# ViktorLiang/GW-Depth

Hardware: AMD Instinct MI355X
Metric: images/sec (train fwd+bwd) 480x640 bs=8/GPU (higher is better)
Workload: dtype bf16; 1 GPU; GW-Depth full model (res50 + DETR 6+6 + 4-scale ReferTransformer + decoder) fwd+17 losses+bwd+clip+AdamW, 480x640, bs=8/GPU, dropout 0.1; global_batch=8, parallelism=dp1, launch=hipgraph, graph_segments=1, grad_buckets=8

## Files before the change

### gw_depth_amd/hip.py

```python
import ctypes
import os

import torch

_HERE = os.path.dirname(os.path.abspath(__file__))
LIB_PATH = os.environ.get("GWD_LIB") or os.path.join(_HERE, "libgwdepth_hip.so")

F32, BF16 = 0, 1
ACT_NONE, ACT_RELU, ACT_GELU, ACT_ELU, ACT_SIGMOID = 0, 1, 2, 3, 4
WS_INORM_GELU, WS_RESAMPLE_BWD, WS_EVAL, WS_PLANE = 0, 1, 2, 3
GATHER_CONV, GATHER_TRANSPOSED, GATHER_UPSAMPLED = 0, 1, 2
RESAMPLE_BILINEAR_AC, RESAMPLE_NEAREST = 0, 1

ENTRY_POINTS = [
    "gwd_version", "gwd_arch", "gwd_conv_forward", "gwd_conv_wgrad", "gwd_weight_prep", "gwd_act_backward",
    "gwd_colsum", "gwd_layernorm_forward", "gwd_layernorm_backward", "gwd_softmax_forward",
    "gwd_softmax_backward", "gwd_silog_sums", "gwd_silog_backward", "gwd_seg_ce_sum", "gwd_seg_ce_backward",
    "gwd_sqnorm", "gwd_adamw_step", "gwd_resample_forward", "gwd_resample_backward", "gwd_avgpool_forward",
    "gwd_avgpool_backward", "gwd_winattn_forward", "gwd_winattn_backward", "gwd_tokattn_forward",
    "gwd_tokattn_backward", "gwd_tokattn_pair_forward", "gwd_tokattn_pair_backward", "gwd_upsample_taps_collapse", "gwd_upsample_taps_fold", "gwd_certain_sample", "gwd_lsap", "gwd_window_map", "gwd_window_map_multi",
    "gwd_inorm_gelu_forward", "gwd_inorm_gelu_backward", "gwd_weight_prep_batch",
    "gwd_point_sample_forward", "gwd_point_sample_backward", "gwd_act_backward_colsum", "gwd_resample_backward_sep",
    "gwd_softmax_masked_forward", "gwd_softmax_scaled_backward", "gwd_query_workspace", "gwd_eval_accumulate", "gwd_colsum_batch", "gwd_conv_wgrad_batch",
    "gwd_conv_wgrad_takes_bias",
    "gwd_plane_loss_forward", "gwd_plane_loss_backward", "gwd_collate",
    "gwd_anchor_depth_forward", "gwd_anchor_depth_backward", "gwd_mha_flash_forward", "gwd_mha_flash_backward",
    "gwd_ref_scores_forward", "gwd_ref_scores_backward", "gwd_ref_mix_forward", "gwd_ref_mix_backward", "gwd_unpad_add_batch", "gwd_stem_pack", "gwd_stem_forward", "gwd_pos_sine", "gwd_silog_finalize", "gwd_psp_pool_forward", "gwd_psp_pool_backward",
    "gwd_match_cost", "gwd_set_losses_forward", "gwd_set_losses_backward", "gwd_set_losses_focal_forward", "gwd_set_losses_focal_backward", "gwd_resample_u8_pass", "gwd_gather2d", "gwd_point_sample_backward_gather", "gwd_point_sample_framed_forward", "gwd_point_sample_framed_backward", "gwd_stride_place", "gwd_color_adjust", "gwd_bmm",
    "gwd_dense_postprocess", "gwd_line_postprocess", "gwd_line_score",
    "gwd_dense_postprocess_resized",
    "gwd_resample_u8_pass_batch", "gwd_gather2d_batch", "gwd_color_adjust_batch",
]


class HipUnavailable(RuntimeError):
    pass


class ConvDesc(ctypes.Structure):
    _fields_ = [("x", ctypes.c_void_p), ("w", ctypes.c_void_p), ("y", ctypes.c_void_p), ("z", ctypes.c_void_p),
                ("scale", ctypes.c_void_p), ("shift", ctypes.c_void_p), ("residual", ctypes.c_void_p),
                ("zero_page", ctypes.c_void_p), ("mult", ctypes.c_void_p), ("gate", ctypes.c_void_p)] + \
               [(n, ctypes.c_int32) for n in ("B", "Hi", "Wi", "Cin", "Ho", "Wo", "Cout", "KH", "KW", "stride", "pad",
                                              "gather", "Hv", "Wv", "act")] + \
               [("act_scale", ctypes.c_float), ("dtype", ctypes.c_int32), ("gate_act", ctypes.c_int32),
                ("ln_mean", ctypes.c_void_p), ("ln_rstd", ctypes.c_void_p), ("ln_C", ctypes.c_int32), ("reserved", ctypes.c_int32),
                ("dbias", ctypes.c_void_p)]


class BmmDesc(ctypes.Structure):
    _fields_ = [("a", ctypes.c_void_p), ("b", ctypes.c_void_p), ("c", ctypes.c_void_p)] + \
               [(n, ctypes.c_int64) for n in ("a_sb0", "a_sb1", "a_ld", "b_sb0", "b_sb1", "b_ld", "c_sb0", "c_sb1", "c_ld")] + \
               [(n, ctypes.c_int32) for n in ("M", "N", "K", "nb0", "nb1", "a_kmajor", "b_kmajor", "c_is_f32_accumulate", "splits")] + \
               [("alpha", ctypes.c_float), ("dtype", ctypes.c_int32)]


class PrepJob(ctypes.Structure):
    _fields_ = [("w", ctypes.c_void_p), ("row_scale", ctypes.c_void_p), ("w_fwd", ctypes.c_void_p), ("w_dgrad", ctypes.c_void_p),
                ("N", ctypes.c_int32), ("taps", ctypes.c_int32), ("C", ctypes.c_int32), ("block0", ctypes.c_int32),
                ("Np", ctypes.c_int32), ("Cg", ctypes.c_int32), ("Cgp", ctypes.c_int32), ("reserved", ctypes.c_int32)]


class UnpadJob(ctypes.Structure):
    _fields_ = [("src", ctypes.c_void_p), ("dst", ctypes.c_void_p), ("N", ctypes.c_int32), ("taps", ctypes.c_int32), ("G", ctypes.c_int32),
# ... 158 lines not shown
        L.gwd_ref_mix_backward.argtypes = [vp, vp, vp, vp, vp, i32, i32, i32, i32, i32, i32, vp]
        L.gwd_tokattn_forward.argtypes = [sp] * 4 + [i64, i32, i32, f32, i32, vp]
        L.gwd_tokattn_backward.argtypes = [sp] * 7 + [i64, i32, i32, f32, i32, vp]
        L.gwd_upsample_taps_collapse.argtypes = [vp, vp, i32, i32, i32, vp]
        L.gwd_upsample_taps_fold.argtypes = [vp, vp, i32, i32, vp]
        L.gwd_tokattn_pair_forward.argtypes = [sp] * 6 + [i64, i32, i32, f32, i32, vp]
        L.gwd_tokattn_pair_backward.argtypes = [sp] * 10 + [i64, i32, i32, f32, i32, vp]
        L.gwd_certain_sample.argtypes = [vp, vp, vp, i32, i32, i32, i32, i32, vp, i32, i32, vp]
        L.gwd_lsap.argtypes = [vp, vp, vp, i32, i32, i32, i32, i32, vp]
        L.gwd_inorm_gelu_forward.argtypes = [vp, vp, vp, vp, vp, i64, i64, i32, i32, ctypes.c_float, i32, vp]
        L.gwd_inorm_gelu_backward.argtypes = [vp, vp, vp, vp, vp, i64, i64, i32, i32, i32, vp]
        L.gwd_query_workspace.argtypes = [i32, ctypes.POINTER(ctypes.c_int64), i32]
        L.gwd_query_workspace.restype = ctypes.c_int64
        L.gwd_eval_accumulate.argtypes = [vp, vp, vp, i64, i64, i64, vp, vp, vp, vp, vp, i32, i64, f32, f32, i32, i32, vp]
        L.gwd_dense_postprocess.argtypes = [vp, vp, i64, i64, i64, vp, vp, vp, vp, i32, i32, i32, f32, f32, i32, i32, vp]
        L.gwd_dense_postprocess_resized.argtypes = [vp, vp, i64, i64, i64, vp, vp, i32, vp, vp, vp] + [i32] * 5 + [f32, f32, i32, i32, vp]
        L.gwd_line_postprocess.argtypes = [vp] * 7 + [i32, i32, i32, f32, vp]
        dp = ctypes.POINTER(ctypes.c_double)
        L.gwd_line_score.argtypes = [vp] * 5 + [dp, i32, dp, i32] + [vp] * 4 + [i32] * 4 + [i64, i64, vp]
        L.gwd_softmax_masked_forward.argtypes = [vp, vp, vp, i64, i32, i64, ctypes.c_float, i32, vp]
        L.gwd_softmax_scaled_backward.argtypes = [vp, vp, vp, i64, i32, ctypes.c_float, i32, vp]
        L.gwd_resample_backward_sep.argtypes = [vp, vp, vp] + [i32] * 9 + [vp]
        L.gwd_act_backward_colsum.argtypes = [vp, vp, vp, vp, i64, i32, i32, ctypes.c_float, vp, i32, vp]
        L.gwd_point_sample_forward.argtypes = [vp, vp, vp, i32, i32, i32, i32, i32, i32, i32, vp]
        L.gwd_point_sample_backward.argtypes = [vp, vp, vp, i32, i32, i32, i32, i32, i32, i32, vp]
        L.gwd_point_sample_backward_gather.argtypes = [vp, vp, vp, i32, i32, i32, i32, i32, i32, i32, vp]
        L.gwd_point_sample_framed_forward.argtypes = [vp, vp, vp, i32, i32, i32, i32, i32, i32, i32, i32, i32, vp]
        L.gwd_point_sample_framed_backward.argtypes = [vp, vp, vp, i32, i32, i32, i32, i32, i32, i32, i32, i32, vp]
        L.gwd_weight_prep_batch.argtypes = [vp, i32, i32, vp, vp]
        L.gwd_window_map.argtypes = [vp, vp, vp, i32, i32, i32, i32, i32, i32, i32, vp]
        L.gwd_window_map_multi.argtypes = [vp, vp, vp, vp, i32, i32, i32, i32, i32, i32, i32, vp]
        L.gwd_sqnorm.argtypes = [vp, vp, i64, vp]
        L.gwd_adamw_step.argtypes = [vp, vp, vp, vp, vp, vp, i64] + [f32] * 9 + [vp]

    @staticmethod
    def _stream(*tensors):
        for t in tensors:
            if t is not None and not t.is_cuda:
                raise HipUnavailable("gw_depth_amd ops run on a HIP device only (got a %s tensor); "
                                     "there is no CPU path" % t.device)
        return ctypes.c_void_p(torch.cuda.current_stream().cuda_stream)

    @staticmethod
    def _check(rc, what):
        if rc != 0:
            raise RuntimeError("%s failed with status %d" % (what, rc))

    def workspace_bytes(self, op, *dims):
        arr = (ctypes.c_int64 * len(dims))(*[int(d) for d in dims])
        n = self.lib.gwd_query_workspace(op, arr, len(dims))
        if n < 0:
            raise ValueError("gwd_query_workspace(%d, %r) -> %d" % (op, dims, n))
        return n

    def version(self):
        return self.lib.gwd_version()

    @staticmethod
    def _desc(x, w, y, dims, z=None, scale=None, shift=None, residual=None, stride=1, pad=0,
              gather=GATHER_CONV, virt=(0, 0), act=ACT_NONE, act_scale=1.0, mult=None, gate=None, gate_act=ACT_NONE, ln=None,
              zero_page=True, dbias=None):
        B, Hi, Wi, Cin, Ho, Wo, Cout, KH, KW = dims
        d = ConvDesc()
        d.x, d.w, d.y, d.z = _ptr(x), _ptr(w), _ptr(y), _ptr(z)
        d.scale, d.shift, d.residual = _ptr(scale), _ptr(shift), _ptr(residual)
        d.zero_page = _zero_page(x.device) if zero_page else None
# ... 381 lines not shown
                                                 dtype_code(ra), self._stream(ra, ref_v, q_new, att)), "gwd_ref_mix_forward")

    def ref_mix_backward(self, att, ref_v, g, d_ra, d_ref_v, H):
        B, T, R = att.shape[0], att.shape[1], att.shape[2]
        self._check(self.lib.gwd_ref_mix_backward(_ptr(att), _ptr(ref_v), _ptr(g), _ptr(d_ra), _ptr(d_ref_v), B, T, R, H,
                                                  ref_v.shape[2] // H, dtype_code(att), self._stream(att, ref_v, g, d_ra, d_ref_v)),
                    "gwd_ref_mix_backward")

    def tokattn_forward(self, q, k, v, o, scale):
        W, N, H, _ = q.shape
        s = [_strided(t) for t in (q, k, v, o)]
        self._check(self.lib.gwd_tokattn_forward(*[ctypes.byref(x) for x in s], W, H, k.shape[3], scale, dtype_code(q),
                                                 self._stream(q, k, v, o)), "gwd_tokattn_forward")

    def tokattn_backward(self, q, k, v, go, gq, gk, gv, scale):
        W, N, H, _ = q.shape
        s = [_strided(t) for t in (q, k, v, go, gq, gk, gv)]
        self._check(self.lib.gwd_tokattn_backward(*[ctypes.byref(x) for x in s], W, H, k.shape[3], scale, dtype_code(q),
                                                  self._stream(q, go, gq)), "gwd_tokattn_backward")

    def upsample_taps_collapse(self, w, wk):
        Cout, KH, KW, Cin = w.shape
        if (KH, KW) != (3, 3) or tuple(wk.shape) != (Cin, 4, 4, Cout) or w.dtype != torch.float32 or not (w.is_contiguous() and wk.is_contiguous()):
            raise ValueError("upsample_taps_collapse: w (Cout,3,3,Cin) fp32 -> wk (Cin,4,4,Cout), both contiguous")
        self._check(self.lib.gwd_upsample_taps_collapse(_ptr(w), _ptr(wk), Cout, Cin, dtype_code(wk), self._stream(w, wk)), "gwd_upsample_taps_collapse")

    def upsample_taps_fold(self, D, dw):
        Cout, KH, KW, Cin = dw.shape
        if (KH, KW) != (3, 3) or tuple(D.shape) != (Cin, 4, 4, Cout) or D.dtype != torch.float32 or dw.dtype != torch.float32 \
                or not (D.is_contiguous() and dw.is_contiguous()):
            raise ValueError("upsample_taps_fold: D (Cin,4,4,Cout) fp32 -> dw (Cout,3,3,Cin) fp32, both contiguous")
        self._check(self.lib.gwd_upsample_taps_fold(_ptr(D), _ptr(dw), Cout, Cin, self._stream(D, dw)), "gwd_upsample_taps_fold")

    def tokattn_pair_forward(self, q, q2, k, v, o, o2, scale):
        W, N, H, _ = q.shape
        s = [_strided(t) for t in (q, q2, k, v, o, o2)]
        rc = self.lib.gwd_tokattn_pair_forward(*[ctypes.byref(x) for x in s], W, H, k.shape[3], scale, dtype_code(q),
                                               self._stream(q, q2, k, v, o, o2))
        if rc == -4:
            return False
        self._check(rc, "gwd_tokattn_pair_forward")
        return True

    def tokattn_pair_backward(self, q, q2, k, v, go, go2, gq, gq2, gk, gv, scale):
        W, N, H, _ = q.shape
        s = [_strided(t) for t in (q, q2, k, v, go, go2, gq, gq2, gk, gv)]
        rc = self.lib.gwd_tokattn_pair_backward(*[ctypes.byref(x) for x in s], W, H, k.shape[3], scale, dtype_code(q),
                                                self._stream(q, go, gq))
        if rc == -4:
            return False
        self._check(rc, "gwd_tokattn_pair_backward")
        return True

    def certain_sample(self, small, large, coords, edges, sample_num):
        B, _, hs, ws = small.shape
        H, W = large.shape[-2:]
        self._check(self.lib.gwd_certain_sample(_ptr(small), _ptr(large), _ptr(coords), B, hs, ws, H, W, _ptr(edges),
                                                edges.numel() - 1, sample_num, self._stream(small, large, coords)),
                    "gwd_certain_sample")

    def bmm(self, a, b, c, M, N, K, a_kmajor=False, b_kmajor=False, alpha=1.0, accumulate=False, splits=1):
        for t in (a, b, c):
            if t.dim() != 4 or t.stride(3) != 1:
                raise ValueError("bmm: 4-D operands with unit inner stride expected")
        nb0, nb1 = c.shape[0], c.shape[1]
        d = BmmDesc()
# ... 209 lines not shown
```

### gw_depth_amd/model.py

```python
import math
import os

import torch
import torch.nn.functional as F
from torch import nn

from . import ops
from .layers import Conv, FrozenBN, LayerNorm, Linear, Mlp, MlpNorm, Seq
from .ops import ACT_ELU, ACT_GELU, ACT_NONE, ACT_RELU, ACT_SIGMOID

WS = 7
HEADS = 16
DEFAULT_FP32_STAGES = ()


class NestedTensor:

    def __init__(self, tensors, mask):
        self.tensors, self.mask = tensors, mask

    def to(self, device):
        return NestedTensor(self.tensors.to(device), None if self.mask is None else self.mask.to(device))

    def decompose(self):
# ... 539 lines not shown

    def __init__(self, c, pools=(16, 8, 4, 2)):
        super().__init__()
        self.pools = pools
        self.firstconv = Seq(_0=ConvLn(c, c, 3), _2=ConvLn(c, 2 * c, 3))
        c2 = 2 * c
        self.layer1 = nn.Sequential(PyrBlock(c2))
        self.layer2 = nn.Sequential(PyrBlock(c2), PyrBlock(c2))
        self.layer3 = nn.Sequential(PyrBlock(c2), PyrBlock(c2))
        self.layer4 = nn.Sequential(PyrBlock(c2))
        for i in range(1, 5):
            setattr(self, f"branch{i}", Seq(_1=ConvLn(c2, c2, 3)))
        self.lastconv = Seq(_0=ConvLn(5 * c2, 2 * c2, 3), _2=Conv(2 * c2, c, 1))

    FORCE_PAD = False

    def padded_width(self, ref):
        c = self.firstconv[0].conv.weight.shape[0]
        if c % 8 and ((ref.dtype == torch.bfloat16 and ref.is_cuda) or self.FORCE_PAD):
            return (c + 31) // 32 * 32
        return c

    def forward(self, x):
        c = self.firstconv[0].conv.weight.shape[0]
        if x.shape[-1] != c:
            return self.forward_padded(x, c)
        x = self.firstconv[2](self.firstconv[0](x, True), True)
        x = self.layer3(self.layer2(self.layer1(x)))
        B, H, W, C = x.shape
        if H < self.pools[0] or W < self.pools[0]:
            x = F.pad(x, (0, 0, 0, max(self.pools[0] - W, 0), 0, max(self.pools[0] - H, 0)))
        x, pooled = ops.psp_pools(x, self.pools)
        ys = [getattr(self, f"branch{i}")[1](p, True) for i, p in enumerate(pooled, start=1)]
        x = self.lastconv[0](ops.pyramid_concat(x, ys), True)
        return ops.conv2d(x, self.lastconv[2].weight)

    def forward_padded(self, x, c):
        r32 = lambda n: (n + 31) // 32 * 32
        cp, c2, c2p, c4, c4p = r32(c), 2 * c, r32(2 * c), 4 * c, r32(4 * c)
        if x.shape[-1] != cp:
            raise ValueError("PyramidLayer: a map of %d or %d channels expected, got %d" % (c, cp, x.shape[-1]))
        x = self.firstconv[2](self.firstconv[0](x, True, geom=(cp, c, cp)), True, geom=(c2p, c, cp))
        g2 = (c2p, c2, c2p)
        for layer in (self.layer1, self.layer2, self.layer3):
            for blk in layer:
                x = blk(x, g2)
        B, H, W, C = x.shape
        if H < self.pools[0] or W < self.pools[0]:
            x = F.pad(x, (0, 0, 0, max(self.pools[0] - W, 0), 0, max(self.pools[0] - H, 0)))
        x, pooled = ops.psp_pools(x, self.pools)
        ys = [getattr(self, f"branch{i}")[1](p, True, geom=g2) for i, p in enumerate(pooled, start=1)]
        x = self.lastconv[0](ops.pyramid_concat(x, ys), True, geom=(c4p, c2, c2p))
        return ops.conv2d_padded(x, self.lastconv[2].weight, 0, (cp, c4, c4p))


class PointBasedPred(nn.Module):

    def __init__(self, dim, tdim, point_num):
        super().__init__()
        self.dim = dim
        self.pre_proj = Linear(dim + tdim, dim)
        self.refer_proj = Linear(dim, dim * 2)
        self.pyramid = PyramidLayer(point_num)

    def forward(self, x, dtok, pre_depth, coords, H, W, pos):
        B = x.shape[0]
        xg_xr = self.refer_proj(self.pre_proj(torch.cat([x, dtok], dim=-1)))
# ... 279 lines not shown
```

### gw_depth_amd/ops.py

```python
import bisect
import os

import torch
import torch.nn.functional as F

from . import hip
from .hip import (ACT_ELU, ACT_GELU, ACT_NONE, ACT_RELU, ACT_SIGMOID, GATHER_CONV, GATHER_TRANSPOSED,
                  GATHER_UPSAMPLED)

__all__ = ["conv2d", "linear", "layer_norm", "softmax_lastdim", "silog_loss", "seg_cross_entropy",
           "ACT_NONE", "ACT_RELU", "ACT_GELU", "ACT_ELU", "ACT_SIGMOID"]


def _lib():
    return hip.library()


class WeightCache:

    def __init__(self, persistent=(), frozen=False):
        self.frozen = bool(frozen)
        self._derived = {}
        self.ranges = sorted((int(a), int(b)) for a, b in persistent)
        self._starts, self._ends, self._merged_from = [], [], -1
# ... 1101 lines not shown
        shapes = []
        for k, y in enumerate(ys):
            y = y.contiguous()
            if y.shape[0] != B or y.shape[3] != C:
                raise ValueError("pyramid_concat: branch %d has shape %r" % (k, tuple(y.shape)))
            lib.resample_forward(y, out[..., (k + 1) * C:(k + 2) * C], B, y.shape[1], y.shape[2], H, W, C, hip.RESAMPLE_BILINEAR_AC)
            shapes.append((y.shape[1], y.shape[2]))
        ctx.cfg = (B, H, W, C, shapes)
        return out

    @staticmethod
    def backward(ctx, g):
        lib = _lib()
        B, H, W, C, shapes = ctx.cfg
        g = g.contiguous()
        grads = [g[..., :C]]
        for k, (h, w) in enumerate(shapes):
            gk = g[..., (k + 1) * C:(k + 2) * C]
            gy = torch.empty((B, h, w, C), dtype=g.dtype, device=g.device)
            tmp = torch.empty(lib.workspace_bytes(hip.WS_RESAMPLE_BWD, B, H, w, C) // 4, dtype=torch.float32, device=g.device)
            if not lib.resample_backward_sep(gk, tmp, gy, B, h, w, H, W, C, hip.RESAMPLE_BILINEAR_AC):
                lib.resample_backward(gk.contiguous(), gy, B, h, w, H, W, C, hip.RESAMPLE_BILINEAR_AC)
            grads.append(gy)
        return tuple(grads)


def pyramid_concat(x, ys):
    C = x.shape[-1]
    if C % 8 or not ys:
        return torch.cat([x] + [upsample_bilinear_ac(y, x.shape[1:3]) for y in ys], dim=-1)
    return _PyramidCatFn.apply(x, *ys)


def upsample_bilinear_ac(x, size):
    return _ResampleFn.apply(x, tuple(size), hip.RESAMPLE_BILINEAR_AC)


def upsample_nearest(x, size):
    return _ResampleFn.apply(x, tuple(size), hip.RESAMPLE_NEAREST)


class _AvgPoolFn(torch.autograd.Function):
    @staticmethod
    def forward(ctx, x, k):
        x = x.contiguous()
        B, H, W, C = x.shape
        y = torch.empty((B, H // k, W // k, C), dtype=x.dtype, device=x.device)
        _lib().avgpool_forward(x, y, B, H, W, C, k)
        ctx.cfg = (B, H, W, C, k)
        return y

    @staticmethod
    def backward(ctx, gy):
        B, H, W, C, k = ctx.cfg
        gx = torch.empty((B, H, W, C), dtype=gy.dtype, device=gy.device)
        _lib().avgpool_backward(gy.contiguous(), gx, B, H, W, C, k)
        return gx, None


def avg_pool(x, k):
    return _AvgPoolFn.apply(x, int(k))


class _WinAttnPackedFn(torch.autograd.Function):

    @staticmethod
# ... 601 lines not shown
```

### include/gwdepth.h

```cpp
#ifndef GWDEPTH_H
#define GWDEPTH_H
#include <stdint.h>

#ifdef __cplusplus
extern "C" {
#endif

#define GWD_VERSION 10

enum { GWD_F32 = 0, GWD_BF16 = 1 };
enum { GWD_ACT_NONE = 0, GWD_ACT_RELU = 1, GWD_ACT_GELU = 2, GWD_ACT_ELU = 3, GWD_ACT_SIGMOID = 4 };
enum {
    GWD_GATHER_CONV = 0,
    GWD_GATHER_TRANSPOSED = 1,
    GWD_GATHER_UPSAMPLED = 2
};

typedef struct {
    const void *x;
    const void *w;
    void *y;
    void *z;
    const float *scale;
    const float *shift;
// ... 183 lines not shown
    const float *src;
    float *dst;
    int32_t N, taps, G, Cg, Cgp;
    int32_t block0;
} gwd_unpad_job;
int gwd_unpad_add_batch(const gwd_unpad_job *jobs, int32_t n_jobs, void *stream);

int gwd_inorm_gelu_forward(const void *a, const void *u, void *y, float *part, float *stat, int64_t B, int64_t L, int32_t C,
                           int32_t S, float eps, int32_t dtype, void *stream);
int gwd_inorm_gelu_backward(const void *gy, const void *u, const float *stat, float *part, void *du, int64_t B, int64_t L,
                            int32_t C, int32_t S, int32_t dtype, void *stream);

int gwd_window_map(const void *src, void *dst, const void *residual, int32_t B, int32_t H, int32_t W, int32_t C, int32_t shift,
                   int32_t gather, int32_t dtype, void *stream);
#define GWD_WINMAP_JOBS 4
int gwd_window_map_multi(const void *const *src, void *const *dst, const void *const *residual, const int32_t *C, int32_t n,
                         int32_t B, int32_t H, int32_t W, int32_t shift, int32_t gather, int32_t dtype, void *stream);

enum { GWD_RESAMPLE_BILINEAR_AC = 0, GWD_RESAMPLE_NEAREST = 1 };
int gwd_resample_forward(const void *x, void *y, int32_t B, int32_t Hs, int32_t Ws, int32_t Ho, int32_t Wo,
                         int32_t C, int32_t mode, int32_t ldy, int32_t dtype, void *stream);
int gwd_resample_backward(const void *gy, void *gx, int32_t B, int32_t Hs, int32_t Ws, int32_t Ho, int32_t Wo,
                          int32_t C, int32_t mode, const void *gate, int32_t gate_act, int32_t dtype, void *stream);
int gwd_resample_backward_sep(const void *gy, float *tmp, void *gx, int32_t B, int32_t Hs, int32_t Ws, int32_t Ho, int32_t Wo,
                              int32_t C, int32_t mode, int32_t ldg, int32_t dtype, void *stream);

int gwd_stride_place(const void *src, const void *residual, void *dst, int32_t B, int32_t H, int32_t W, int32_t Ho, int32_t Wo, int32_t C,
                     int32_t stride, int32_t dtype, void *stream);

int gwd_psp_pool_forward(const void *x, void *p16, void *p8, void *p4, void *p2, int32_t B, int32_t H, int32_t W, int32_t C,
                         int32_t dtype, void *stream);
int gwd_psp_pool_backward(const void *g_pass, const void *g16, const void *g8, const void *g4, const void *g2, void *gx, int32_t B,
                          int32_t H, int32_t W, int32_t C, int32_t ldg, int32_t dtype, void *stream);
int gwd_avgpool_forward(const void *x, void *y, int32_t B, int32_t H, int32_t W, int32_t C, int32_t k,
                        int32_t dtype, void *stream);
int gwd_avgpool_backward(const void *gy, void *gx, int32_t B, int32_t H, int32_t W, int32_t C, int32_t k,
                         int32_t dtype, void *stream);

int gwd_sqnorm(const float *g, double *sq, int64_t n, void *stream);
int gwd_adamw_step(float *p, const float *g, float *m, float *v, void *p_bf16, const double *sq,
                   int64_t n, float lr, float beta1, float beta2, float eps, float weight_decay,
                   float bias_corr1, float bias_corr2, float max_norm, float grad_scale, void *stream);

#define GWD_EVAL_NSUM 10
int gwd_eval_accumulate(const void *pred_depth, const float *gt_depth, const void *seg_logits, int64_t seg_sb,
                        int64_t seg_sp, int64_t seg_sc, const int64_t *seg_gt, void *workspace, double *measures,
                        double *running, int64_t *confusion, int32_t B, int64_t HW, float min_depth,
                        float max_depth, int32_t depth_dtype, int32_t seg_dtype, void *stream);

int gwd_dense_postprocess(const void *depth, const void *seg_logits, int64_t seg_sb, int64_t seg_sp, int64_t seg_sc,
                          const int32_t *sizes, float *depth_out, uint16_t *depth_mm, uint8_t *label, int32_t B, int32_t H,
                          int32_t W, float min_depth, float max_depth, int32_t depth_dtype, int32_t seg_dtype, void *stream);

int gwd_dense_postprocess_resized(const void *depth, const void *seg_logits, int64_t seg_sb, int64_t seg_sp, int64_t seg_sc,
                                  const int32_t *sizes, const int32_t *frame_sizes, int32_t twin, float *depth_out,
                                  uint16_t *depth_mm, uint8_t *label, int32_t B, int32_t H, int32_t W, int32_t Fh, int32_t Fw,
                                  float min_depth, float max_depth, int32_t depth_dtype, int32_t seg_dtype, void *stream);

int gwd_line_postprocess(const float *logits, const float *lines, const int32_t *sizes, float *scores, float *lines_px,
                         int32_t *order, int32_t *count, int32_t B, int32_t Q, int32_t ld, float thresh, void *stream);

int gwd_line_score(const float *logits, const float *lines, const int32_t *sizes, const float *gt, const int32_t *gt_count,
                   const double *nms_thresholds, int32_t T, const double *sap_thresholds, int32_t S, uint8_t *flag,
                   double *kept_lines, float *score, int32_t *gt_seen, int32_t B, int32_t Q, int32_t ld, int32_t G,
                   int64_t capacity, int64_t slot, void *stream);

// ... 78 lines not shown
```

Before: 257.0 images/s.

## Apply PSP tail conv to low-res pyramid branches before upsampling

The PSP head's final 3x3 conv over the concatenation of the input and upsampled pooled branches is split. The three lowest-resolution branches are convolved at their pooled resolution into per-tap 1x1 outputs, and a fused kernel then bilinearly upsamples those taps, adds the high-res partial conv, and applies LayerNorm (+GELU). The backward pass mirrors this with a gather kernel and a weight-grad fold. This avoids materialising the full-resolution concatenation and running the 3x3 conv over its upsampled channels, at the cost of extra kernels, new code and bf16 rounding-order differences.

```diff
diff --git a/gw_depth_amd/csrc/pyrtail.hip b/gw_depth_amd/csrc/pyrtail.hip
--- /dev/null
+++ b/gw_depth_amd/csrc/pyrtail.hip
@@ -0,0 +1,378 @@
+#include "common.h"
+
+namespace {
+
+constexpr int PT_TH = 8, PT_TW = 8;
+constexpr int PT_CH = 32;
+constexpr int PT_MAXCHUNK = 10;
+constexpr int PT_MAXR = 5, PT_MAXC = 5;
+constexpr int PT_MAXPOS = PT_MAXR * PT_MAXC;
+constexpr int PT_TAB = 128;
+constexpr int PT_SPLIT = 4;
+
+struct PyrBranches {
+    void *p[GWD_PYR_MAX_BRANCHES];
+    int h[GWD_PYR_MAX_BRANCHES], w[GWD_PYR_MAX_BRANCHES];
+    int start[GWD_PYR_MAX_BRANCHES + 1];
+    int n;
+};
+
+__device__ __forceinline__ float pt_scale(int in, int out) { return out > 1 ? (float)(in - 1) / (float)(out - 1) : 0.f; }
+
+__device__ __forceinline__ float pt_weight(int o, int s, int in, float scale) {
+    const float f = scale * o;
+    const int i0 = (int)f, i1 = i0 + (i0 < in - 1);
+    const float l = f - i0;
+    return (i0 == s ? 1.f - l : 0.f) + (i1 == s ? l : 0.f);
+}
+
+template <typename T> struct Vec8;
+template <> struct alignas(16) Vec8<__bf16> { __bf16 e[8]; };
+template <> struct alignas(16) Vec8<float> { float e[8]; };
+
+template <typename T> struct Raw8;
+template <> struct Raw8<__bf16> { uint4 a; };
+template <> struct Raw8<float> { uint4 a, b; };
+
+template <typename T>
+__device__ __forceinline__ void fma8(float (&acc)[8], float wgt, const Vec8<T> &v) {
+#pragma unroll
+    for (int e = 0; e < 8; ++e) acc[e] = fmaf(wgt, to_f32(v.e[e]), acc[e]);
+}
+
+template <typename T>
+__global__ __launch_bounds__(256) void pyr_tail_fwd_kernel(const T *__restrict__ part, const PyrBranches br, const float *__restrict__ gamma,
+                                                           const float *__restrict__ beta, T *__restrict__ z, T *__restrict__ y,
+                                                           float *__restrict__ mean, float *__restrict__ rstd, int H, int W, int N, int gelu) {
+    __shared__ Vec8<T> smz[PT_MAXPOS * 36];
+    __shared__ Vec8<float> smh[PT_MAXR * 3 * PT_TW * 4];
+    const int t = threadIdx.x, q = t & 3, pix = t >> 2;
+    const int ntx = (W + PT_TW - 1) / PT_TW, nty = (H + PT_TH - 1) / PT_TH;
+    const long vb = xcd_grouped_block(blockIdx.x, gridDim.x, 2 * ntx);
+    const int px0 = (int)(vb % ntx) * PT_TW, py0 = (int)((vb / ntx) % nty) * PT_TH, b = (int)(vb / ((long)ntx * nty));
+    const int pxl = pix & (PT_TW - 1);
+    const int px = px0 + pxl, py = py0 + pix / PT_TW;
+    const bool inside = px < W && py < H;
+    const int nch = N / PT_CH;
+    float acc[PT_MAXCHUNK][8];
+#pragma unroll
+    for (int j = 0; j < PT_MAXCHUNK; ++j)
+#pragma unroll
+        for (int e = 0; e < 8; ++e) acc[j][e] = 0.f;
+    const int ya = max(py0 - 1, 0), yb = min(py0 + PT_TH, H - 1), xa = max(px0 - 1, 0), xb = min(px0 + PT_TW, W - 1);
+    for (int k = 0; k < br.n; ++k) {
+        const int h = br.h[k], w = br.w[k];
+        const float sh = pt_scale(h, H), sw = pt_scale(w, W);
+        const int rlo = (int)(sh * ya), rhi = min((int)(sh * yb) + 1, h - 1);
+        const int clo = (int)(sw * xa), chi = min((int)(sw * xb) + 1, w - 1);
+        const int nc = min(chi - clo + 1, PT_MAXC), nr = min(rhi - rlo + 1, PT_MAXR);
+        const T *Zk = (const T *)br.p[k] + (size_t)b * h * w * 9 * N;
+        static_assert(PT_MAXPOS * 36 <= 4 * 256, "four window places a thread");
+        const int nitem = nr * nc * 36;
+        auto place = [&](int u) {
+            const int i = min(t + u * 256, nitem - 1);
+            const int pos = i / 36, rem = i - pos * 36;
+            return (((rlo + pos / nc) * w + clo + pos % nc) * 9 + (rem >> 2)) * N + (rem & 3) * 8;
+        };
+        const int zoff0 = place(0), zoff1 = place(1), zoff2 = place(2), zoff3 = place(3);
+        typedef Raw8<T> R8;
+        R8 pre0 = *(const R8 *)(Zk + zoff0), pre1 = *(const R8 *)(Zk + zoff1), pre2 = *(const R8 *)(Zk + zoff2), pre3 = *(const R8 *)(Zk + zoff3);
+        R8 *smr = (R8 *)smz;
+#pragma unroll
+        for (int j = 0; j < PT_MAXCHUNK; ++j) {
+            if (j < nch) {
+                if (t < nitem) smr[t] = pre0;
+                if (t + 256 < nitem) smr[t + 256] = pre1;
+                if (t + 512 < nitem) smr[t + 512] = pre2;
+                if (t + 768 < nitem) smr[t + 768] = pre3;
+                __syncthreads();
+                if (j + 1 < nch) {
+                    const T *Zn = Zk + (j + 1) * PT_CH;
+                    pre0 = *(const R8 *)(Zn + zoff0);
+                    pre1 = *(const R8 *)(Zn + zoff1);
+                    pre2 = *(const R8 *)(Zn + zoff2);
+                    pre3 = *(const R8 *)(Zn + zoff3);
+                }
+                for (int i = t; i < nr * 3 * PT_TW * 4; i += 256) {
+                    const int lane = i & 3, xl = (i >> 2) & (PT_TW - 1), rt = i / (PT_TW * 4);
+                    const int rr = rt / 3, ty = rt - rr * 3;
+                    Vec8<float> hv;
+#pragma unroll
+                    for (int e = 0; e < 8; ++e) hv.e[e] = 0.f;
+#pragma unroll
+                    for (int tx = 0; tx < 3; ++tx) {
+                        const int xx = px0 + xl + tx - 1;
+                        if (xx < 0 || xx >= W) continue;
+                        const float fx = sw * xx;
+                        const int c0 = (int)fx, c1 = c0 + (c0 < w - 1);
+                        const float lx = fx - c0, hx = 1.f - lx;
+                        const int tq = (ty * 3 + tx) * 4 + lane;
+                        fma8<T>(hv.e, hx, smz[(rr * nc + min(c0 - clo, PT_MAXC - 1)) * 36 + tq]);
+                        fma8<T>(hv.e, lx, smz[(rr * nc + min(c1 - clo, PT_MAXC - 1)) * 36 + tq]);
+                    }
+                    smh[i] = hv;
+                }
+                __syncthreads();
+                if (inside) {
+#pragma unroll
+                    for (int ty = 0; ty < 3; ++ty) {
+                        const int yy = py + ty - 1;
+                        if (yy < 0 || yy >= H) continue;
+                        const float fy = sh * yy;
+                        const int r0 = (int)fy, r1 = r0 + (r0 < h - 1);
+                        const float ly = fy - r0, hy = 1.f - ly;
+                        fma8<float>(acc[j], hy, smh[((min(r0 - rlo, PT_MAXR - 1) * 3 + ty) * PT_TW + pxl) * 4 + q]);
+                        fma8<float>(acc[j], ly, smh[((min(r1 - rlo, PT_MAXR - 1) * 3 + ty) * PT_TW + pxl) * 4 + q]);
+                    }
+                }
+            }
+        }
+    }
+    const size_t row = ((size_t)b * H + (inside ? py : 0)) * W + (inside ? px : 0);
+    float s = 0.f;
+#pragma unroll
+    for (int j = 0; j < PT_MAXCHUNK; ++j) {
+        if (j < nch && inside) {
+            const size_t off = row * N + j * PT_CH + q * 8;
+            const Vec8<T> pv = *(const Vec8<T> *)(part + off);
+            Vec8<T> zv;
+#pragma unroll
+            for (int e = 0; e < 8; ++e) {
+                zv.e[e] = from_f32<T>(acc[j][e] + to_f32(pv.e[e]));
+                acc[j][e] = to_f32(zv.e[e]);
+                s += acc[j][e];
+            }
+            if (z) *(Vec8<T> *)(z + off) = zv;
+        }
+    }
+    s += __shfl_xor(s, 1, 64);
+    s += __shfl_xor(s, 2, 64);
+    const float mu = s / (float)N;
+    float v2 = 0.f;
+#pragma unroll
+    for (int j = 0; j < PT_MAXCHUNK; ++j) {
+        if (j < nch) {
+#pragma unroll
+            for (int e = 0; e < 8; ++e) {
+                const float d = acc[j][e] - mu;
+                v2 += d * d;
+            }
+        }
+    }
+    v2 += __shfl_xor(v2, 1, 64);
+    v2 += __shfl_xor(v2, 2, 64);
+    const float rs = rsqrtf(v2 / (float)N + 1e-5f);
+    if (!inside) return;
+    if (q == 0) {
+        mean[row] = mu;
+        rstd[row] = rs;
+    }
+#pragma unroll
+    for (int j = 0; j < PT_MAXCHUNK; ++j) {
+        if (j < nch) {
+            const int ch = j * PT_CH + q * 8;
+            Vec8<T> ov;
+#pragma unroll
+            for (int e = 0; e < 8; ++e) {
+                float o = (acc[j][e] - mu) * rs * gamma[ch + e] + beta[ch + e];
+                if (gelu) o = gelu_t<T>(o);
+                ov.e[e] = from_f32<T>(o);
+            }
+            *(Vec8<T> *)(y + row * N + ch) = ov;
+        }
+    }
+}
+
+template <typename T>
+__global__ __launch_bounds__(256) void pyr_tail_bwd_kernel(const T *__restrict__ gz, const PyrBranches br, int H, int W, int N) {
+    __shared__ float sm[(PT_SPLIT - 1) * 9 * (PT_MAXCHUNK * 4) * 8];
+    __shared__ float tabx[PT_TAB * 3], taby[PT_TAB * 3];
+    const int lanes = N / 8, lane = threadIdx.x % lanes, grp = threadIdx.x / lanes;
+    int k = 0;
+    while (k + 1 < br.n && (int)blockIdx.x >= br.start[k + 1]) ++k;
+    const int h = br.h[k], w = br.w[k];
+    const int local = (int)xcd_grouped_block(blockIdx.x - br.start[k], br.start[k + 1] - br.start[k], 2 * w);
+    const int c = local % w, r = (local / w) % h, b = local / (w * h);
+    const float sh = pt_scale(h, H), sw = pt_scale(w, W);
+    int ylo = 0, yhi = H - 1, xlo = 0, xhi = W - 1;
+    if (sh > 0.f) {
+        ylo = max(0, (int)floorf((r - 1) / sh) - 2);
+        yhi = min(H - 1, (int)ceilf((r + 1) / sh) + 2);
+    }
+    if (sw > 0.f) {
+        xlo = max(0, (int)floorf((c - 1) / sw) - 2);
+        xhi = min(W - 1, (int)ceilf((c + 1) / sw) + 2);
+    }
+    auto wx_of = [&](int xx, int tx) {
+        const int sx = xx + tx - 1;
+        return (sx >= 0 && sx < W) ? pt_weight(sx, c, w, sw) : 0.f;
+    };
+    while (xlo < xhi && wx_of(xlo, 0) == 0.f && wx_of(xlo, 1) == 0.f && wx_of(xlo, 2) == 0.f) ++xlo;
+    while (xhi > xlo && wx_of(xhi, 0) == 0.f && wx_of(xhi, 1) == 0.f && wx_of(xhi, 2) == 0.f) --xhi;
+    auto wy_of = [&](int yy, int ty) {
+        const int sy = yy + ty - 1;
+        return (sy >= 0 && sy < H) ? pt_weight(sy, r, h, sh) : 0.f;
+    };
+    const bool tab = xhi - xlo < PT_TAB && yhi - ylo < PT_TAB;
+    if (tab) {
+        for (int i = threadIdx.x; i < (xhi - xlo + 1) * 3; i += blockDim.x) tabx[i] = wx_of(xlo + i / 3, i % 3);
+        for (int i = threadIdx.x; i < (yhi - ylo + 1) * 3; i += blockDim.x) taby[i] = wy_of(ylo + i / 3, i % 3);
+        __syncthreads();
+    }
+    float acc[9][8];
+#pragma unroll
+    for (int i = 0; i < 9; ++i)
+#pragma unroll
+        for (int e = 0; e < 8; ++e) acc[i][e] = 0.f;
+    const T *gb = gz + (size_t)b * H * W * N + lane * 8;
+    for (int yy = ylo + grp; yy <= yhi; yy += PT_SPLIT) {
+        float wy[3];
+#pragma unroll
+        for (int ty = 0; ty < 3; ++ty) wy[ty] = tab ? taby[(yy - ylo) * 3 + ty] : wy_of(yy, ty);
+        if (wy[0] == 0.f && wy[1] == 0.f && wy[2] == 0.f) continue;
+        float rowsum[3][8];
+#pragma unroll
+        for (int i = 0; i < 3; ++i)
+#pragma unroll
+            for (int e = 0; e < 8; ++e) rowsum[i][e] = 0.f;
+#pragma unroll 4
+        for (int xx = xlo; xx <= xhi; ++xx) {
+            float wx[3];
+#pragma unroll
+            for (int tx = 0; tx < 3; ++tx) wx[tx] = tab ? tabx[(xx - xlo) * 3 + tx] : wx_of(xx, tx);
+            const Vec8<T> v = *(const Vec8<T> *)(gb + ((size_t)yy * W + xx) * N);
+#pragma unroll
+            for (int tx = 0; tx < 3; ++tx) fma8<T>(rowsum[tx], wx[tx], v);
+        }
+#pragma unroll
+        for (int ty = 0; ty < 3; ++ty)
+#pragma unroll
+            for (int tx = 0; tx < 3; ++tx)
+#pragma unroll
+                for (int e = 0; e < 8; ++e) acc[ty * 3 + tx][e] = fmaf(wy[ty], rowsum[tx][e], acc[ty * 3 + tx][e]);
+    }
+    if (grp > 0) {
+#pragma unroll
+        for (int i = 0; i < 9; ++i)
+#pragma unroll
+            for (int e = 0; e < 8; ++e) sm[(((grp - 1) * 9 + i) * lanes + lane) * 8 + e] = acc[i][e];
+    }
+    __syncthreads();
+    if (grp == 0) {
+        T *G = (T *)br.p[k] + ((size_t)(b * h + r) * w + c) * 9 * N + lane * 8;
+#pragma unroll
+        for (int i = 0; i < 9; ++i) {
+            Vec8<T> ov;
+#pragma unroll
+            for (int e = 0; e < 8; ++e) {
+                float v = acc[i][e];
+#pragma unroll
+                for (int g = 0; g < PT_SPLIT - 1; ++g) v += sm[((g * 9 + i) * lanes + lane) * 8 + e];
+                ov.e[e] = from_f32<T>(v);
+            }
+            *(Vec8<T> *)(G + (size_t)i * N) = ov;
+        }
+    }
+}
+
+struct PyrFold {
+    const float *lo[GWD_PYR_MAX_BRANCHES];
+};
+__global__ __launch_bounds__(256) void pyr_tail_fold_kernel(const float *__restrict__ d_hi, const PyrFold lo, float *__restrict__ dw, int N,
+                                                            int C2, int nbr, int nlow, int64_t total) {
+    const int64_t i = (int64_t)blockIdx.x * 256 + threadIdx.x;
+    if (i >= total) return;
+    const int Cw = (1 + nbr) * C2, Chi = (1 + nbr - nlow) * C2;
+    const int ch = (int)(i % Cw);
+    const int64_t nt = i / Cw;
+    const int tap = (int)(nt % 9), n = (int)(nt / 9);
+    const int g = ch / C2, ci = ch - g * C2;
+    float v;
+    if (g == 0) v = d_hi[nt * Chi + ci];
+    else if (g <= nlow) v = lo.lo[g - 1][((size_t)tap * N + n) * C2 + ci];
+    else v = d_hi[nt * Chi + (g - nlow) * C2 + ci];
+    dw[i] += v;
+}
+
+int check_branches(const int32_t *hk, const int32_t *wk, int nb, int H, int W) {
+    for (int k = 0; k < nb; ++k) {
+        if (hk[k] <= 0 || wk[k] <= 0 || hk[k] > H || wk[k] > W) return -1;
+    }
+    return 0;
+}
+
+}
+
+extern "C" int gwd_pyr_tail_forward(const void *part, const void *const *Z, const int32_t *hk, const int32_t *wk, int32_t nb,
+                                    const float *gamma, const float *beta, void *z, void *y, float *mean, float *rstd, int32_t B,
+                                    int32_t H, int32_t W, int32_t N, int32_t gelu, int32_t dtype, void *stream) {
+    if (!part || !Z || !hk || !wk || !gamma || !beta || !y || !mean || !rstd || B <= 0 || H <= 0 || W <= 0 || N <= 0) return -1;
+    if (nb < 1 || nb > GWD_PYR_MAX_BRANCHES || check_branches(hk, wk, nb, H, W)) return -1;
+    if (dtype != GWD_BF16 && dtype != GWD_F32) return -2;
+    if (N % PT_CH || N > PT_CH * PT_MAXCHUNK) return -4;
+    PyrBranches br = {};
+    br.n = nb;
+    for (int k = 0; k < nb; ++k) {
+        if (!Z[k]) return -1;
+        const double sh = H > 1 ? (double)(hk[k] - 1) / (H - 1) : 0.0, sw = W > 1 ? (double)(wk[k] - 1) / (W - 1) : 0.0;
+        int nr = (int)(sh * (PT_TH + 1) * (1.0 + 1e-6)) + 3, nc = (int)(sw * (PT_TW + 1) * (1.0 + 1e-6)) + 3;
+        nr = nr < hk[k] ? nr : hk[k];
+        nc = nc < wk[k] ? nc : wk[k];
+        if (nr > PT_MAXR || nc > PT_MAXC) return -4;
+        br.p[k] = const_cast<void *>(Z[k]);
+        br.h[k] = hk[k];
+        br.w[k] = wk[k];
+    }
+    const int64_t nblk = (int64_t)B * ((W + PT_TW - 1) / PT_TW) * ((H + PT_TH - 1) / PT_TH);
+    if (nblk >= (1LL << 31)) return -7;
+    const int grid = (int)nblk;
+    if (dtype == GWD_BF16)
+        pyr_tail_fwd_kernel<__bf16><<<grid, 256, 0, (hipStream_t)stream>>>((const __bf16 *)part, br, gamma, beta, (__bf16 *)z, (__bf16 *)y, mean,
+                                                                           rstd, H, W, N, gelu);
+    else
+        pyr_tail_fwd_kernel<float><<<grid, 256, 0, (hipStream_t)stream>>>((const float *)part, br, gamma, beta, (float *)z, (float *)y, mean, rstd,
+                                                                          H, W, N, gelu);
+    GWD_CHECK_LAUNCH();
+    return 0;
+}
+
+extern "C" int gwd_pyr_tail_backward(const void *gz, void *const *G, const int32_t *hk, const int32_t *wk, int32_t nb, int32_t B, int32_t H,
+                                     int32_t W, int32_t N, int32_t dtype, void *stream) {
+    if (!gz || !G || !hk || !wk || B <= 0 || H <= 0 || W <= 0 || N <= 0) return -1;
+    if (nb < 1 || nb > GWD_PYR_MAX_BRANCHES || check_branches(hk, wk, nb, H, W)) return -1;
+    if (dtype != GWD_BF16 && dtype != GWD_F32) return -2;
+    if (N % 8 || N > PT_CH * PT_MAXCHUNK) return -4;
+    PyrBranches br = {};
+    br.n = nb;
+    int64_t blocks = 0;
+    for (int k = 0; k < nb; ++k) {
+        if (!G[k]) return -1;
+        br.p[k] = G[k];
+        br.h[k] = hk[k];
+        br.w[k] = wk[k];
+        br.start[k] = (int)blocks;
+        blocks += (int64_t)B * hk[k] * wk[k];
+        if (blocks >= (1LL << 31)) return -7;
+    }
+    br.start[nb] = (int)blocks;
+    const int threads = N / 8 * PT_SPLIT;
+    if (dtype == GWD_BF16) pyr_tail_bwd_kernel<__bf16><<<(int)blocks, threads, 0, (hipStream_t)stream>>>((const __bf16 *)gz, br, H, W, N);
+    else pyr_tail_bwd_kernel<float><<<(int)blocks, threads, 0, (hipStream_t)stream>>>((const float *)gz, br, H, W, N);
+    GWD_CHECK_LAUNCH();
+    return 0;
+}
+
+extern "C" int gwd_pyr_tail_fold_wgrad(const float *d_hi, const float *const *d_low, int32_t nlow, float *dw, int32_t N, int32_t C2,
+                                       int32_t nbr, void *stream) {
+    if (!d_hi || !d_low || !dw || N <= 0 || C2 <= 0 || nbr < 1 || nbr > GWD_PYR_MAX_BRANCHES || nlow < 1 || nlow > nbr) return -1;
+    PyrFold lo = {};
+    for (int k = 0; k < nlow; ++k) {
+        if (!d_low[k]) return -1;
+        lo.lo[k] = d_low[k];
+    }
+    const int64_t total = (int64_t)N * 9 * (1 + nbr) * C2;
+    if ((total + 255) / 256 >= (1LL << 31)) return -7;
+    pyr_tail_fold_kernel<<<(int)((total + 255) / 256), 256, 0, (hipStream_t)stream>>>(d_hi, lo, dw, N, C2, nbr, nlow, total);
+    GWD_CHECK_LAUNCH();
+    return 0;
+}
diff --git a/gw_depth_amd/hip.py b/gw_depth_amd/hip.py
--- a/gw_depth_amd/hip.py
+++ b/gw_depth_amd/hip.py
@@ -30,6 +30,7 @@
     "gwd_dense_postprocess", "gwd_line_postprocess", "gwd_line_score",
     "gwd_dense_postprocess_resized",
     "gwd_resample_u8_pass_batch", "gwd_gather2d_batch", "gwd_color_adjust_batch",
+    "gwd_pyr_tail_forward", "gwd_pyr_tail_backward", "gwd_pyr_tail_fold_wgrad",
 ]
 
 
@@ -254,6 +255,10 @@
         L.gwd_window_map_multi.argtypes = [vp, vp, vp, vp, i32, i32, i32, i32, i32, i32, i32, vp]
         L.gwd_sqnorm.argtypes = [vp, vp, i64, vp]
         L.gwd_adamw_step.argtypes = [vp, vp, vp, vp, vp, vp, i64] + [f32] * 9 + [vp]
+        pvp, pi32 = ctypes.POINTER(ctypes.c_void_p), ctypes.POINTER(ctypes.c_int32)
+        L.gwd_pyr_tail_forward.argtypes = [vp, pvp, pi32, pi32, i32] + [vp] * 6 + [i32] * 6 + [vp]
+        L.gwd_pyr_tail_backward.argtypes = [vp, pvp, pi32, pi32, i32] + [i32] * 5 + [vp]
+        L.gwd_pyr_tail_fold_wgrad.argtypes = [vp, pvp, i32, vp, i32, i32, i32, vp]
 
     @staticmethod
     def _stream(*tensors):
@@ -701,6 +706,48 @@
             raise ValueError("upsample_taps_fold: D (Cin,4,4,Cout) fp32 -> dw (Cout,3,3,Cin) fp32, both contiguous")
         self._check(self.lib.gwd_upsample_taps_fold(_ptr(D), _ptr(dw), Cout, Cin, self._stream(D, dw)), "gwd_upsample_taps_fold")
 
+    PYR_MAX_BRANCHES = 4
+
+    @staticmethod
+    def _pyr_branches(maps, B, N, like):
+        if not 1 <= len(maps) <= HipLibrary.PYR_MAX_BRANCHES:
+            raise ValueError("pyr_tail: 1 to %d low-resolution branches, got %d" % (HipLibrary.PYR_MAX_BRANCHES, len(maps)))
+        for m in maps:
+            if m.dim() != 5 or m.shape[0] != B or m.shape[3] != 9 or m.shape[4] != N or m.dtype != like.dtype or not m.is_contiguous():
+                raise ValueError("pyr_tail: a product map is (B,h,w,9,N) contiguous in the map's dtype, got %r" % (tuple(m.shape),))
+        ptrs = (ctypes.c_void_p * len(maps))(*[m.data_ptr() for m in maps])
+        hk = (ctypes.c_int32 * len(maps))(*[m.shape[1] for m in maps])
+        wk = (ctypes.c_int32 * len(maps))(*[m.shape[2] for m in maps])
+        return ptrs, hk, wk
+
+    def pyr_tail_forward(self, part, Zs, gamma, beta, z, y, mean, rstd, gelu):
+        B, H, W, N = part.shape
+        ptrs, hk, wk = self._pyr_branches(Zs, B, N, part)
+        rc = self.lib.gwd_pyr_tail_forward(_ptr(part), ptrs, hk, wk, len(Zs), _ptr(gamma), _ptr(beta), _ptr(z), _ptr(y), _ptr(mean), _ptr(rstd),
+                                           B, H, W, N, int(bool(gelu)), dtype_code(part), self._stream(part, y, *Zs))
+        if rc == -4:
+            return False
+        self._check(rc, "gwd_pyr_tail_forward")
+        return True
+
+    def pyr_tail_backward(self, gz, Gs):
+        B, H, W, N = gz.shape
+        ptrs, hk, wk = self._pyr_branches(Gs, B, N, gz)
+        self._check(self.lib.gwd_pyr_tail_backward(_ptr(gz), ptrs, hk, wk, len(Gs), B, H, W, N, dtype_code(gz), self._stream(gz, *Gs)),
+                    "gwd_pyr_tail_backward")
+
+    def pyr_tail_fold_wgrad(self, d_hi, d_low, dw, C2):
+        N, Cw, nlow = dw.shape[0], dw.shape[-1], len(d_low)
+        nbr = Cw // C2 - 1
+        ok = dw.dtype == torch.float32 and dw.is_contiguous() and tuple(dw.shape) == (N, 3, 3, (1 + nbr) * C2) and 1 <= nlow <= nbr \
+            and d_hi.dtype == torch.float32 and d_hi.is_contiguous() and d_hi.numel() == N * 9 * (1 + nbr - nlow) * C2 \
+            and all(d.dtype == torch.float32 and d.is_contiguous() and d.numel() == 9 * N * C2 for d in d_low)
+        if not ok:
+            raise ValueError("pyr_tail_fold_wgrad: contiguous fp32 tensors in the documented shapes expected")
+        ptrs = (ctypes.c_void_p * nlow)(*[d.data_ptr() for d in d_low])
+        self._check(self.lib.gwd_pyr_tail_fold_wgrad(_ptr(d_hi), ptrs, nlow, _ptr(dw), N, C2, nbr, self._stream(d_hi, dw, *d_low)),
+                    "gwd_pyr_tail_fold_wgrad")
+
     def tokattn_pair_forward(self, q, q2, k, v, o, o2, scale):
         W, N, H, _ = q.shape
         s = [_strided(t) for t in (q, q2, k, v, o, o2)]
diff --git a/gw_depth_amd/model.py b/gw_depth_amd/model.py
--- a/gw_depth_amd/model.py
+++ b/gw_depth_amd/model.py
@@ -595,7 +595,11 @@
             x = F.pad(x, (0, 0, 0, max(self.pools[0] - W, 0), 0, max(self.pools[0] - H, 0)))
         x, pooled = ops.psp_pools(x, self.pools)
         ys = [getattr(self, f"branch{i}")[1](p, True) for i, p in enumerate(pooled, start=1)]
-        x = self.lastconv[0](ops.pyramid_concat(x, ys), True)
+        tail = self.lastconv[0]
+        if ops.PYRAMID_TAIL_LOWRES and tuple(self.pools) == (16, 8, 4, 2) and ops.pyramid_tail_supported(x, ys, tail.conv.weight):
+            x = ops.pyramid_tail(x, ys, tail.conv.weight, tail.layer_norm.weight, tail.layer_norm.bias, True)
+        else:
+            x = tail(ops.pyramid_concat(x, ys), True)
         return ops.conv2d(x, self.lastconv[2].weight)
 
     def forward_padded(self, x, c):
diff --git a/gw_depth_amd/ops.py b/gw_depth_amd/ops.py
--- a/gw_depth_amd/ops.py
+++ b/gw_depth_amd/ops.py
@@ -1157,6 +1157,120 @@
     return _PyramidCatFn.apply(x, *ys)
 
 
+PYRAMID_TAIL_LOWRES = True
+PYRAMID_TAIL_NLOW = 3
+
+
+class _Ctx:
+    """Stands in for an autograd context where a Function's forward / backward pair is reused inside another Function."""
+
+
+class _PyramidTailFn(torch.autograd.Function):
+
+    @staticmethod
+    def forward(ctx, x, w, gamma, beta, gelu, nlow, w_sink, ln_sinks, *ys):
+        lib = _lib()
+        B, H, W, C2 = x.shape
+        N = w.shape[0]
+        nbr = len(ys)
+        if tuple(w.shape) != (N, 3, 3, (1 + nbr) * C2) or not 1 <= nlow <= nbr:
+            raise ValueError("pyramid_tail: weight %r does not fit %d branches of %d channels" % (tuple(w.shape), nbr, C2))
+        dt = x.dtype
+        lows = [y.contiguous() for y in ys[:nlow]]
+        cctx = _Ctx()
+        cat = _PyramidCatFn.forward(cctx, x, *ys[nlow:]) if nlow < nbr else x.contiguous()
+        Chi = cat.shape[-1]
+        w_hi = derived_weight(w, ("pyr_tail_hi", nlow), lambda: torch.cat([w.detach()[..., :C2], w.detach()[..., (1 + nlow) * C2:]], dim=-1))
+        w_lo = [derived_weight(w, ("pyr_tail_lo", k), lambda k=k: w.detach()[..., (k + 1) * C2:(k + 2) * C2].permute(1, 2, 0, 3)
+                               .reshape(9 * N, 1, 1, C2).contiguous()) for k in range(nlow)]
+        part = torch.empty((B, H, W, N), dtype=dt, device=x.device)
+        dims = (B, H, W, Chi, H, W, N, 3, 3)
+        lib.conv_forward(cat, _weight_for(w_hi, None, dt), part, dims, stride=1, pad=1)
+        Zs = []
+        for y, wl in zip(lows, w_lo):
+            h, wd = y.shape[1], y.shape[2]
+            Z = torch.empty((B, h, wd, 9, N), dtype=dt, device=x.device)
+            lib.conv_forward(y, _weight_for(wl, None, dt), Z.view(B, h, wd, 9 * N), (B, h, wd, C2, h, wd, 9 * N, 1, 1), stride=1, pad=0)
+            Zs.append(Z)
+        need_grad = any(ctx.needs_input_grad)
+        out = torch.empty_like(part)
+        z = torch.empty_like(part) if need_grad else None
+        mean = torch.empty(B * H * W, dtype=torch.float32, device=x.device)
+        rstd = torch.empty(B * H * W, dtype=torch.float32, device=x.device)
+        g, b = gamma.detach(), beta.detach()
+        if lib.pyr_tail_forward(part, Zs, g, b, z, out, mean, rstd, gelu) is False:
+            raise ValueError("pyramid_tail: no kernel for N = %d with branches %r" % (N, [tuple(y.shape[1:3]) for y in lows]))
+        if need_grad:
+            ctx.save_for_backward(cat, w, z, g, b, mean, rstd, *lows)
+        ctx.cfg = (dims, bool(gelu), nlow, nbr, C2, w_sink, ln_sinks, cctx, w_hi, w_lo)
+        return out
+
+    @staticmethod
+    def backward(ctx, gy):
+        lib = _lib()
+        cat, w, z, g, b, mean, rstd, *lows = ctx.saved_tensors
+        dims, gelu, nlow, nbr, C2, w_sink, ln_sinks, cctx, w_hi, w_lo = ctx.cfg
+        B, H, W, Chi, _, _, N, _, _ = dims
+        dt = cat.dtype
+        rows = B * H * W
+        gz = torch.empty_like(z)
+        dg = db = None
+        if ln_sinks is not None:
+            (dg, h1), (db, h2) = ln_sinks
+        else:
+            dg = torch.zeros(N, dtype=torch.float32, device=z.device)
+            db = torch.zeros(N, dtype=torch.float32, device=z.device)
+        lib.layernorm_backward(gy.contiguous(), z, g, b, mean, rstd, gz, dg, db, rows, N, gelu)
+        if ln_sinks is not None:
+            for h in (h1, h2):
+                if h is not None:
+                    h()
+        g_cat = torch.empty_like(cat)
+        lib.conv_forward(gz, _weight_transposed(w_hi, None, dt), g_cat, (B, H, W, N, H, W, Chi, 3, 3), stride=1, pad=1, gather=GATHER_TRANSPOSED)
+        g_high = list(_PyramidCatFn.backward(cctx, g_cat)) if nlow < nbr else [g_cat]
+        Gs = [torch.empty((B, y.shape[1], y.shape[2], 9, N), dtype=dt, device=z.device) for y in lows]
+        lib.pyr_tail_backward(gz, Gs)
+        g_low = []
+        for y, G, wl in zip(lows, Gs, w_lo):
+            h, wd = y.shape[1], y.shape[2]
+            gyk = torch.empty_like(y)
+            lib.conv_forward(G.view(B, h, wd, 9 * N), _weight_transposed(wl, None, dt), gyk, (B, h, wd, 9 * N, h, wd, C2, 1, 1), stride=1, pad=0,
+                             gather=GATHER_TRANSPOSED)
+            g_low.append(gyk)
+        gw = None
+        if ctx.needs_input_grad[1]:
+            d_hi = WGRADS.scratch((N, 3, 3, Chi), z.device)
+            d_lo = [WGRADS.scratch((9 * N, 1, 1, C2), z.device) for _ in lows]
+            if w_sink is None:
+                gw = torch.zeros(w.shape, dtype=torch.float32, device=w.device)
+            dst = gw if w_sink is None else w_sink[0].view(w.shape)
+
+            def fold(d_hi=d_hi, d_lo=d_lo, dst=dst, hook=None if w_sink is None else w_sink[1]):
+                lib.pyr_tail_fold_wgrad(d_hi, d_lo, dst, C2)
+                if hook is not None:
+                    hook()
+
+            WGRADS.add(cat, gz, d_hi, dims, dict(stride=1, pad=1))
+            for i, (y, G, d) in enumerate(zip(lows, Gs, d_lo)):
+                h, wd = y.shape[1], y.shape[2]
+                WGRADS.add(y, G.view(B, h, wd, 9 * N), d, (B, h, wd, C2, h, wd, 9 * N, 1, 1), dict(stride=1, pad=0),
+                           fold if i == len(lows) - 1 else None)
+        grads = g_high[:1] + [gw] + ([None, None] if ln_sinks is not None else [dg, db]) + [None] * 4 + g_low + g_high[1:]
+        return tuple(grads)
+
+
+def pyramid_tail_supported(x, ys, w):
+    N, C2 = w.shape[0], x.shape[-1]
+    return (x.is_cuda and not getattr(_lib(), "is_fake", False) and x.dtype in (torch.float32, torch.bfloat16) and C2 % 8 == 0
+            and N % 32 == 0 and N <= 320 and len(ys) > PYRAMID_TAIL_NLOW >= 1 and tuple(w.shape[1:]) == (3, 3, (1 + len(ys)) * C2))
+
+
+def pyramid_tail(x, ys, w, gamma, beta, gelu=False, nlow=None):
+    sg, sb = _sink(gamma), _sink(beta)
+    ln_sinks = (sg, sb) if (sg is not None and sb is not None) else None
+    return _PyramidTailFn.apply(x, w, gamma, beta, bool(gelu), int(PYRAMID_TAIL_NLOW if nlow is None else nlow), _sink(w), ln_sinks, *ys)
+
+
 def upsample_bilinear_ac(x, size):
     return _ResampleFn.apply(x, tuple(size), hip.RESAMPLE_BILINEAR_AC)
 
diff --git a/include/gwdepth.h b/include/gwdepth.h
--- a/include/gwdepth.h
+++ b/include/gwdepth.h
@@ -239,6 +239,14 @@
                          int32_t dtype, void *stream);
 int gwd_psp_pool_backward(const void *g_pass, const void *g16, const void *g8, const void *g4, const void *g2, void *gx, int32_t B,
                           int32_t H, int32_t W, int32_t C, int32_t ldg, int32_t dtype, void *stream);
+#define GWD_PYR_MAX_BRANCHES 4
+int gwd_pyr_tail_forward(const void *part, const void *const *Z, const int32_t *hk, const int32_t *wk, int32_t nb,
+                         const float *gamma, const float *beta, void *z, void *y, float *mean, float *rstd, int32_t B,
+                         int32_t H, int32_t W, int32_t N, int32_t gelu, int32_t dtype, void *stream);
+int gwd_pyr_tail_backward(const void *gz, void *const *G, const int32_t *hk, const int32_t *wk, int32_t nb, int32_t B, int32_t H,
+                          int32_t W, int32_t N, int32_t dtype, void *stream);
+int gwd_pyr_tail_fold_wgrad(const float *d_hi, const float *const *d_low, int32_t nlow, float *dw, int32_t N, int32_t C2,
+                            int32_t nbr, void *stream);
 int gwd_avgpool_forward(const void *x, void *y, int32_t B, int32_t H, int32_t W, int32_t C, int32_t k,
                         int32_t dtype, void *stream);
 int gwd_avgpool_backward(const void *gy, void *gx, int32_t B, int32_t H, int32_t W, int32_t C, int32_t k,
```

Measured after the change: 262.1 images/s (median of 6 runs). +2.0%, better.
